# JaredWinkens/sdr-iq-visualizer

Measured on AMD Instinct MI355X. Metric: complex64 IQ Msamples/s through windowed FFT+log-PSD, N=4096; % HBM3E peak, higher is better.
Workload: dtype f32

## Files before the change

experiments/f4k_order/timeline.py:

```python
import argparse
import ctypes
import json
import os
import sys

REPO = os.path.dirname(os.path.dirname(os.path.dirname(os.path.abspath(__file__))))
sys.path.insert(0, REPO)
import torch
import numpy as np
from bench import warm_up_by_time
from sdr_iq_visualizer_amd import _ffi
from sdr_iq_visualizer_amd.spectrum import SpectrumPlan

NFFT = 4096
TICK_NS = 10.0
BIN_MS = 0.5


def analyse(rec, n_frames):
    t = rec[:, 0].astype(np.uint64) | (rec[:, 1].astype(np.uint64) << np.uint64(32))
    assert (t > 0).all(), "frames without a record"
    assert np.array_equal(rec[:, 2], np.arange(n_frames, dtype=np.uint32)), "a record names another frame than its own"
    wg = rec[:, 3].astype(np.int64)
    grid = int(wg.max()) + 1
# ... 7 lines not shown
    n_bins = int(np.ceil((ms.max() + 1e-9) / BIN_MS))
    cut = np.searchsorted(ms[order], np.arange(n_bins + 1) * BIN_MS, side="left")
    cut[-1] = n_frames
    for b in range(n_bins):
        hi = (b + 1) * BIN_MS
        idx = order[cut[b]:cut[b + 1]]
        if idx.size == 0:
            continue
        reached[wg[idx]] = frame[idx]
        active = (last_ms >= hi) & (reached >= 0)
        front = int(reached.max())
        lag = int(front - reached[active].min()) if active.any() else 0
        bins.append({"ms": round(b * BIN_MS, 2), "frames": int(idx.size), "span": int(frame[idx].max() - frame[idx].min()),
                     "lag_frames": lag, "lag_grids": round(lag / grid, 2)})
    return {"grid": grid, "launch_ms_by_records": round(float(ms.max()), 3), "bins": bins}


def main():
    ap = argparse.ArgumentParser()
    ap.add_argument("--out", required=True)
    ap.add_argument("--frames", type=int, default=1 << 20)
    ap.add_argument("--short", type=int, default=65536)
    ap.add_argument("--pairs", type=int, default=3)
    a = ap.parse_args()
    lib = _ffi.lib()
    _ffi.require_device(0)
    set_tl = lib.sdrk_f4k_timeline
    set_tl.argtypes, set_tl.restype = [ctypes.c_void_p], ctypes.c_int
    os.environ["SDRK_F4K_PARTS"] = "1"
    d_in = ctypes.c_void_p()
    _ffi.check(lib.sdrk_dev_alloc(0, a.frames * NFFT * 8, ctypes.byref(d_in)))
    outs = []
    for _ in range(a.pairs):
        p = ctypes.c_void_p()
        _ffi.check(lib.sdrk_dev_alloc(0, a.frames * NFFT * 4, ctypes.byref(p)))
        outs.append(p)
    _ffi.check(lib.sdrk_synth_fill(0, 1234, 0, a.frames, NFFT, d_in, None))
    tl = torch.zeros((a.frames, 4), dtype=torch.int32, device="cuda")
    os.makedirs(os.path.dirname(os.path.abspath(a.out)), exist_ok=True)
    with open(a.out, "a") as out:
        for order in ("stride", "ticket"):
            os.environ["SDRK_F4K_ORDER"] = order
            with SpectrumPlan(NFFT, window="hann", device=0) as plan:
                warm_up_by_time(lambda: plan.exec_device_timed(d_in.value, a.frames, outs[0].value, 1))
                for i, p in enumerate(outs):
                    for n in (a.frames, a.short):
                        plan.exec_device_timed(d_in.value, n, p.value, 1)
                        tl.zero_()
                        torch.cuda.synchronize()
                        assert set_tl(tl.data_ptr()) == 0
                        ms = plan.exec_device_timed(d_in.value, n, p.value, 1)
                        assert set_tl(None) == 0
                        rec = tl[:n].cpu().numpy().view(np.uint32)
                        r = {"order": order, "pair": i, "frames": n, "launch_ms_by_events": round(float(ms), 4), **analyse(rec, n)}
                        out.write(json.dumps(r) + "\n")
                        out.flush()
                        print(f"== {order} pair {i} frames {n}: {r['launch_ms_by_events']} ms by events, "
                              f"{r['launch_ms_by_records']} ms first to last issue, grid {r['grid']}")
                        for b in r["bins"]:
                            print(f"   {b['ms']:5.2f} ms  frames {b['frames']:7d}  span {b['span']:8d}  lag {b['lag_frames']:8d} "
                                  f"frames = {b['lag_grids']:7.2f} grids", flush=True)
    for p in outs:
        lib.sdrk_dev_free(0, p)
    lib.sdrk_dev_free(0, d_in)

# ... 4 lines not shown
```

sdr-iq-visualizer_amd/csrc/aux_kernels.hip:

```cpp
#include "kernels.h"
#include "synth_hash.h"

namespace sdrk {

__global__ __launch_bounds__(256) void synth_fill_kernel(uint32_t seed, uint64_t first_frame,
                                                         size_t n_frames, int nfft,
                                                         float4* __restrict__ out) {
    const size_t pairs_per_frame = (size_t)nfft / 2;
    const size_t total = n_frames * pairs_per_frame;
    for (size_t i = (size_t)blockIdx.x * blockDim.x + threadIdx.x; i < total;
         i += (size_t)gridDim.x * blockDim.x) {
        const size_t f = i / pairs_per_frame;
        const uint32_t n = (uint32_t)(i - f * pairs_per_frame) * 2u;
        const uint64_t F = first_frame + f;
        const uint32_t base = synth_frame_base(seed, F);
        int i0, q0, i1, q1;
        synth_codes(base, n, i0, q0);
        synth_codes(base, n + 1u, i1, q1);
        float4 v;
        v.x = (float)i0;
        v.y = (float)q0;
        v.z = (float)i1;
        v.w = (float)q1;
        out[i] = v;
// ... 112 lines not shown
__global__ __launch_bounds__(256) void copy_1to1_kernel(const v4f* __restrict__ in, v4f* __restrict__ out, size_t n_vec) {
    const size_t stride = (size_t)gridDim.x * 256 * 4;
    for (size_t i = (size_t)blockIdx.x * 1024 + threadIdx.x; i < n_vec; i += stride) {
        v4f v[4];
#pragma unroll
        for (int j = 0; j < 4; ++j)
            if (i + 256 * j < n_vec) v[j] = __builtin_nontemporal_load(&in[i + 256 * j]);
#pragma unroll
        for (int j = 0; j < 4; ++j)
            if (i + 256 * j < n_vec) __builtin_nontemporal_store(v[j], &out[i + 256 * j]);
    }
}

hipError_t launch_copy_1to1(const void* d_in, void* d_out, size_t bytes, int num_cus, int blocks_per_cu, hipStream_t stream) {
    const size_t n_vec = bytes / 16;
    if (n_vec == 0) return hipSuccess;
    size_t blocks = (n_vec + 1023) / 1024;
    if (blocks > (size_t)num_cus * blocks_per_cu) blocks = (size_t)num_cus * blocks_per_cu;
    hipLaunchKernelGGL(copy_1to1_kernel, dim3((unsigned)blocks), dim3(256), 0, stream, static_cast<const v4f*>(d_in),
                       static_cast<v4f*>(d_out), n_vec);
    return hipGetLastError();
}

hipError_t launch_power_mean(const void* d_spec, size_t n_frames, int nfft, float scale, float* d_out,
                             hipStream_t stream) {
    hipLaunchKernelGGL(power_mean_kernel, dim3((nfft + 255) / 256), dim3(256), 0, stream,
                       static_cast<const float2*>(d_spec), n_frames, nfft, scale, d_out);
    return hipGetLastError();
}

}
```

sdr-iq-visualizer_amd/csrc/fft4096.hip:

```cpp
#include "fft4096_core.h"

namespace sdrk {

#ifdef SDRK_F4K_TIMELINE
__device__ uint4* f4k_timeline_buf = nullptr;
#define F4K_TIMELINE_LOAD() uint4* const f4k_tl = f4k_timeline_buf
#define F4K_TIMELINE_MARK(fr)                                                                                   \
    do {                                                                                                        \
        if (f4k_tl && tid == 0 && (fr) < n_frames) {                                                            \
            const unsigned long long f4k_t = wall_clock64();                                                    \
            f4k_tl[fr] = make_uint4((unsigned)f4k_t, (unsigned)(f4k_t >> 32), (unsigned)(fr), blockIdx.x);      \
        }                                                                                                       \
    } while (0)
#else
#define F4K_TIMELINE_LOAD() (void)0
#define F4K_TIMELINE_MARK(fr) (void)0
#endif

template <bool HAS_WINDOW, int EPILOGUE>
__global__ __launch_bounds__(F4K_THREADS, F4K_WAVES) void fft4096_kernel(
    const float2* __restrict__ iq, size_t frame_stride, void* __restrict__ out_raw,
    size_t n_frames, const float* __restrict__ window, const float2* __restrict__ tw4096,
    float eps, int shift) {
    typedef F4kInC64 In;
// ... 94 lines not shown
        if (last_of_ticket && tid == 0) {
            ticket_slot[par] = drawn;
            drawn = __hip_atomic_fetch_add(head, 1u, __ATOMIC_RELAXED, __HIP_MEMORY_SCOPE_AGENT);
        }
        In::to_owners(nxt, lds, tid);
        cf v[16];
#pragma unroll
        for (int j = 0; j < 16; ++j) v[j] = In::widen(nxt[j]);
        issue(nxt, nx);
        f4k_windowed_transform<HAS_WINDOW>(v, lds, tw256, tw1, lds_win, A, tid);
        size_t after = nx + 1;
        if (last_of_ticket) {
            after = tn;
            tn = first_of(__builtin_amdgcn_readfirstlane(ticket_slot[par]));
            par ^= 1;
        }
        f4k_store_row<EPILOGUE>(v, frame_rsrc(static_cast<char*>(out_raw) + cur * (size_t)(F4K_N * OUT_ELEM), F4K_N * OUT_ELEM),
                                voff_out, xor_k2, eps);
        cur = nx;
        nx = after;
    }
}

unsigned f4k_max_blocks(int num_cus) { return f4k_grid(num_cus, F4K_WAVES, (size_t)-1); }

hipError_t launch_fft4096(const LaunchArgs& a) {
    if (a.n_frames == 0) return hipSuccess;
    dim3 g(f4k_grid(a.num_cus, F4K_WAVES, a.n_frames)), b(F4K_THREADS);
    const float2* iq = static_cast<const float2*>(a.d_iq);
    const float2* tw = static_cast<const float2*>(a.d_twiddle);
#define SDRK_LAUNCH(W, E)                                                                            \
    hipLaunchKernelGGL((fft4096_kernel<W, E>), g, b, 0, a.stream, iq, a.frame_stride, a.d_out,           \
                       a.n_frames, a.d_window, tw, a.eps, a.shift)
    if (a.epilogue == EPI_LOGPSD) {
        if (a.d_window) SDRK_LAUNCH(true, EPI_LOGPSD); else SDRK_LAUNCH(false, EPI_LOGPSD);
    } else {
        if (a.d_window) SDRK_LAUNCH(true, EPI_COMPLEX); else SDRK_LAUNCH(false, EPI_COMPLEX);
    }
#undef SDRK_LAUNCH
    return hipGetLastError();
}

hipError_t launch_fft4096_ticket(const LaunchArgs& a, unsigned* d_heads, const sdrk_host::F4kTicketBases& bases,
                                 sdrk_host::F4kTicketForm form, unsigned grid) {
    if (a.n_frames == 0) return hipSuccess;
    if (!d_heads || grid == 0 || grid % sdrk_host::F4K_TICKET_MAX_HEADS || !sdrk_host::f4k_ticket_form_ok(form)) return hipErrorInvalidValue;
    dim3 g(grid), b(F4K_THREADS);
    const float2* iq = static_cast<const float2*>(a.d_iq);
    const float2* tw = static_cast<const float2*>(a.d_twiddle);
#define SDRK_LAUNCH(W, E)                                                                            \
    hipLaunchKernelGGL((fft4096_ticket_kernel<W, E>), g, b, 0, a.stream, iq, a.frame_stride, a.d_out,    \
                       a.n_frames, a.d_window, tw, a.eps, a.shift, d_heads, bases, form)
    if (a.epilogue == EPI_LOGPSD) {
        if (a.d_window) SDRK_LAUNCH(true, EPI_LOGPSD); else SDRK_LAUNCH(false, EPI_LOGPSD);
    } else {
        if (a.d_window) SDRK_LAUNCH(true, EPI_COMPLEX); else SDRK_LAUNCH(false, EPI_COMPLEX);
    }
#undef SDRK_LAUNCH
    return hipGetLastError();
}

}

#ifdef SDRK_F4K_TIMELINE
extern "C" int sdrk_f4k_timeline(void* d_records) {
    uint4* p = static_cast<uint4*>(d_records);
    return (int)hipMemcpyToSymbol(HIP_SYMBOL(sdrk::f4k_timeline_buf), &p, sizeof p);
}
#endif
```

sdr-iq-visualizer_amd/csrc/kernels.h:

```cpp
#pragma once
#include <hip/hip_runtime.h>
#include <stddef.h>
#include <stdint.h>

#include <atomic>

#include "f4k_ticket.h"

#ifdef SDRK_PHASE_MARKS
#define SDRK_PHASE(name) asm volatile("; SDRK_PHASE " name ::: "memory")
#else
#define SDRK_PHASE(name) do { } while (0)
#endif

namespace sdrk {

enum Epilogue : int {
    EPI_LOGPSD = 0,
    EPI_COMPLEX = 1,
    EPI_BLU_MUL = 2,
    EPI_BLU_POST_LOG = 3,
    EPI_BLU_POST_C64 = 4,
};

struct LaunchArgs {
    const void* d_iq = nullptr;
    size_t frame_stride = 0;
    void* d_out = nullptr;
    size_t n_frames = 0;
    int nfft = 0;
// ... 26 lines not shown

__device__ __forceinline__ float logpsd_db_fast(float p) {
    return __builtin_amdgcn_logf(p) * 3.01029995663981195213f;
}

#endif

inline hipError_t ensure_dynamic_lds(const void* kernel, size_t lds_bytes, std::atomic<uint64_t>& mask) {
    if (lds_bytes <= 64 * 1024) return hipSuccess;
    int dev = 0;
    hipError_t e = hipGetDevice(&dev);
    if (e != hipSuccess) return e;
    const uint64_t bit = (dev >= 0 && dev < 64) ? (uint64_t)1 << dev : 0;
    if (bit && (mask.load(std::memory_order_acquire) & bit)) return hipSuccess;
    e = hipFuncSetAttribute(kernel, hipFuncAttributeMaxDynamicSharedMemorySize, (int)lds_bytes);
    if (e == hipSuccess && bit) mask.fetch_or(bit, std::memory_order_release);
    return e;
}

hipError_t launch_fft4096(const LaunchArgs& a);
unsigned f4k_max_blocks(int num_cus);
hipError_t launch_fft4096_ticket(const LaunchArgs& a, unsigned* d_heads, const sdrk_host::F4kTicketBases& bases,
                                 sdrk_host::F4kTicketForm form, unsigned grid);
hipError_t launch_fft_small(const LaunchArgs& a);
bool fft_lds_supports(int nfft);
hipError_t launch_fft_lds(const LaunchArgs& a);
bool fft_tiled2_split(int nfft, int* log2a, int* log2m);
hipError_t launch_fft_tiled2(const LaunchArgs& a);
bool fft_tiled2_has_mip(int nfft, int epilogue);
hipError_t launch_synth_fill(uint32_t seed, uint64_t first_frame, size_t n_frames, int nfft,
                             void* d_iq, hipStream_t stream);

size_t fused64k_ring_bytes();
size_t fused64k_ctrl_words();
unsigned fused64k_sets(int num_cus);
hipError_t launch_fused64k(const LaunchArgs& a, void* d_ring, unsigned* d_ctrl);
bool blu_fused_supports(int M);
hipError_t launch_blu_fused(const void* d_iq, size_t frame_stride, size_t n_frames, int N, int M, const float* d_window,
                            const void* d_chirp, const void* d_bspec, const void* d_twM, float eps, int shift,
                            int epilogue, void* d_out, int num_cus, hipStream_t s);
hipError_t launch_blu_pre(const void* d_iq, size_t frame_stride, size_t n_frames, int N, int M, const float* d_window,
                          const void* d_chirp, void* d_a, int num_cus, hipStream_t s, bool compact = false);
hipError_t launch_blu_mul(const void* d_A, const void* d_B, size_t n_frames, int M, void* d_out, int num_cus,
                          hipStream_t s);
hipError_t launch_blu_post(const void* d_Y, const void* d_chirp, size_t n_frames, int N, int M, float eps, int shift,
                           int epilogue, void* d_out, int num_cus, hipStream_t s);
hipError_t launch_row_features(const float* d_rows, size_t n_rows, int nfft, int rank, float gamma, int min_distance,
                               int max_peaks, double* d_stats, double* d_thr, int* d_idx, int* d_cnt, int num_cus,
                               hipStream_t s);
hipError_t launch_feature_finalize(const double* d_stats, const double* d_thr, const int* d_idx, const int* d_cnt,
                                   size_t n_rows, int nfft, float gamma, int max_peaks, const double* d_freqs,
                                   double* d_out, hipStream_t s);
hipError_t launch_fft4096_features(const LaunchArgs& a, int rank, float gamma, int min_distance, int max_peaks,
                                   double* d_stats, double* d_thr, int* d_idx, int* d_cnt);
hipError_t launch_row_peaks(const float* d_rows, size_t n_rows, int nfft, const double* d_thr, int min_distance,
                            int max_peaks, int* d_idx, int* d_count, hipStream_t s);
hipError_t launch_decimate_rows(const float* d_ring, int nfft, int maxlen, int start_slot, int n_rows, int factor,
                                int mode, float* d_out, hipStream_t stream);
hipError_t launch_decimate_mip(const float* d_mip_ring, int nfft, int maxlen, int start_slot, int n_rows, int factor,
                               float* d_out, hipStream_t stream);
hipError_t launch_stream_mix(const void* d_in, void* d_out, size_t n_frames4096, int num_cus, hipStream_t stream);
hipError_t launch_copy_1to1(const void* d_in, void* d_out, size_t bytes, int num_cus, int blocks_per_cu, hipStream_t stream);
hipError_t launch_power_mean(const void* d_spec, size_t n_frames, int nfft, float scale, float* d_out,
                             hipStream_t stream);

}
```

sdr-iq-visualizer_amd/csrc/plan_internal.h:

```cpp
#pragma once
#include <hip/hip_runtime.h>

#include <cstddef>
#include <cstdint>
#include <map>
#include <mutex>
#include <utility>
#include <vector>

#include "../../include/sdrk.h"
#include "kernels.h"

namespace sdrk_host {
constexpr int HOST_SLOTS = 3;
struct ChunkOut {
    enum Rows {
        None,
        Pooled,
        Direct,
        Kernel,
        Planes,
    } rows = None;
    void* user = nullptr;
    size_t bytes = 0;
// ... 67 lines not shown
    bool fused64k = false, fused_auto = false, fused_broken = false;
    void* d_fused_ring = nullptr;
    unsigned* d_fused_ctrl = nullptr;
    unsigned* h_fused_err = nullptr;
    unsigned fused_launches = 0, fused_pending = 0;
    int precision = 32;
    double eps64 = 0.0;
    double* d_window64 = nullptr;
    double* d_tw64 = nullptr;
    void* d_scratch64 = nullptr;
    sdrk_host::Staging ci16;
    sdrk_host::Staging integ;
    float* d_pfb_h = nullptr;
    int pfb_taps = 0;
    int pfb_assign = 0;
    sdrk_host::Staging pfb;
    float2* d_fir_h = nullptr;
    int fir_taps = 0;
    int fir_assign = 0;
    int f4k_order = sdrk_host::F4K_ORDER_AUTO;
    sdrk_host::F4kTicketForm f4k_form = sdrk_host::F4K_TICKET_FORM;
    unsigned* d_f4k_heads = nullptr;
    sdrk_host::F4kTicketBases f4k_bases = {};
    hipEvent_t f4k_ev = nullptr;
    hipStream_t f4k_last = nullptr;
    bool f4k_recorded = false;
    size_t f4k_parts = 0;
};

namespace sdrk_host {

constexpr size_t SMALL_IN_BYTES = 256 << 10;
constexpr size_t HOST_CHUNK_BYTES = 16 << 20;
constexpr size_t ZERO_COPY_MAX_BYTES = 32 << 20;
constexpr unsigned FUSED_MAILBOX = 64;
constexpr size_t FUSED_AUTO_MIN_FRAMES = 512;

int fail(int status, const char* fmt, ...) __attribute__((format(printf, 2, 3)));

#define HIP_TRY(expr)                                                                                                   \
    do {                                                                                                                \
        hipError_t e__ = (expr);                                                                                        \
        if (e__ != hipSuccess)                                                                                          \
            return ::sdrk_host::fail(e__ == hipErrorOutOfMemory ? SDRK_ERR_NOMEM : SDRK_ERR_HIP,                        \
                                     "%s failed: %s (%s:%d)", #expr, hipGetErrorString(e__), __FILE__, __LINE__);       \
    } while (0)
// ... 196 lines not shown
```

sdr-iq-visualizer_amd/csrc/sdrk_plan.hip:

```cpp
#include "../../include/sdrk.h"

#include <hip/hip_runtime.h>

#include <cmath>
#include <cstdio>
#include <cstdlib>
#include <cstring>
#include <dlfcn.h>
#include <mutex>
#include <new>
#include <vector>

#include "f4k_split.h"
#include "kernels.h"
#include "plan_internal.h"

using namespace sdrk_host;

namespace sdrk_host {

struct EpiArgs {
    const float2* tab = nullptr;
    int n_out = 0;
    float eps = 0.0f;
// ... 129 lines not shown
            if (st != SDRK_OK) return st;
            e = sdrk::launch_blu_mul(p->d_blu_b, p->d_blu_bspec, nf, M, p->d_blu_a, p->num_cus, stream);
            if (e != hipSuccess) break;
            st = plan_launch(p->blu_inner, p->d_blu_a, nf, (size_t)M, p->d_blu_b, sdrk::EPI_COMPLEX, stream);
            if (st != SDRK_OK) return st;
            e = sdrk::launch_blu_post(p->d_blu_b, p->d_blu_chirp, nf, N, M, p->eps, p->shift, epilogue,
                                      static_cast<char*>(d_out) + f0 * (size_t)N * out_elem, p->num_cus, stream);
            if (e != hipSuccess) break;
        }
    } else if (p->nfft == 4096) {
        const size_t max_blocks = sdrk::f4k_max_blocks(p->num_cus);
        const bool ticket = p->d_f4k_heads && f4k_ticket_takes(p->f4k_order, max_blocks, n_frames, F4K_TICKET_DEFAULT);
        size_t parts = p->f4k_parts ? p->f4k_parts : (ticket ? f4k_ticket_parts(n_frames) : f4k_split_parts(n_frames));
        if (p->f4k_parts && parts > n_frames) parts = n_frames ? n_frames : 1;
        const size_t per = (n_frames + parts - 1) / parts;
        const size_t out_elem = epilogue == sdrk::EPI_LOGPSD ? sizeof(float) : sizeof(float2);
        if (ticket && p->f4k_recorded && p->f4k_last != stream) e = hipStreamWaitEvent(stream, p->f4k_ev, 0);
        for (size_t f0 = 0; f0 < n_frames && e == hipSuccess; f0 += per) {
            a.d_iq = static_cast<const float2*>(d_iq) + f0 * frame_stride;
            a.d_out = static_cast<char*>(d_out) + f0 * (size_t)4096 * out_elem;
            a.n_frames = n_frames - f0 < per ? n_frames - f0 : per;
            if (ticket) {
                const unsigned grid = f4k_ticket_grid(max_blocks, a.n_frames);
                e = sdrk::launch_fft4096_ticket(a, p->d_f4k_heads, p->f4k_bases, p->f4k_form, grid);
                if (e == hipSuccess) f4k_ticket_advance(p->f4k_form, p->f4k_bases, a.n_frames, grid);
            } else {
                e = sdrk::launch_fft4096(a);
            }
        }
        if (ticket && e == hipSuccess) {
            e = hipEventRecord(p->f4k_ev, stream);
            p->f4k_last = stream;
            p->f4k_recorded = true;
        }
    } else if (sdrk::fft_lds_supports(p->nfft))
        e = sdrk::launch_fft_lds(a);
    else if (p->nfft < 4096)
        e = sdrk::launch_fft_small(a);
    else if (takes_fused(p, call_frames) && !d_mip && epilogue <= sdrk::EPI_COMPLEX) {
        FusedGate& gate = fused_gate(p->device);
        std::lock_guard<std::mutex> lk(gate.mu);
        if (gate.ev && gate.last_stream != stream && gate.recorded) e = hipStreamWaitEvent(stream, gate.ev, 0);
        if (e == hipSuccess) e = sdrk::launch_fused64k(a, p->d_fused_ring, p->d_fused_ctrl);
        if (e == hipSuccess)
            e = hipMemcpyAsync(p->h_fused_err + 16 * (p->fused_launches++ % FUSED_MAILBOX), p->d_fused_ctrl,
                               16 * sizeof(unsigned), hipMemcpyDeviceToHost, stream);
        if (e == hipSuccess && gate.ev) {
            e = hipEventRecord(gate.ev, stream);
// ... 163 lines not shown
            const double ang = M_PI * (double)r / (double)nfft;
            c[n] = make_float2((float)std::cos(ang), (float)std::sin(ang));
            b[n] = c[n];
            if (n) b[M - n] = c[n];
        }
        PLAN_TRY(hipMalloc((void**)&p->d_blu_chirp, sizeof(float2) * nfft));
        PLAN_TRY(hipMemcpy(p->d_blu_chirp, c.data(), sizeof(float2) * nfft, hipMemcpyHostToDevice));
        PLAN_TRY(hipMalloc((void**)&p->d_blu_a, (one_kernel ? 1 : frames) * (size_t)M * sizeof(float2)));
        if (!one_kernel) PLAN_TRY(hipMalloc((void**)&p->d_blu_b, frames * (size_t)M * sizeof(float2)));
        PLAN_TRY(hipMalloc((void**)&p->d_blu_bspec, (size_t)M * sizeof(float2)));
        PLAN_TRY(hipMemcpy(p->d_blu_a, b.data(), sizeof(float2) * M, hipMemcpyHostToDevice));
        st2 = plan_launch(p->blu_inner, p->d_blu_a, 1, (size_t)M, p->d_blu_bspec, sdrk::EPI_COMPLEX, p->stream);
        if (st2 != SDRK_OK) { sdrk_plan_destroy(p); return st2; }
        PLAN_TRY(hipStreamSynchronize(p->stream));
        *out = p;
        return SDRK_OK;
    }
    if (nfft <= 16384) {
        std::vector<float2> t(nfft);
        for (int m = 0; m < nfft; ++m) t[m] = twiddle(m, nfft);
        PLAN_TRY(hipMalloc((void**)&p->d_twiddle, sizeof(float2) * nfft));
        PLAN_TRY(hipMemcpy(p->d_twiddle, t.data(), sizeof(float2) * nfft, hipMemcpyHostToDevice));
        if (nfft == 4096) {
            if (const char* env = getenv("SDRK_F4K_ORDER"))
                p->f4k_order = env[0] == 't' ? F4K_ORDER_TICKET : (env[0] == 's' ? F4K_ORDER_STRIDE : F4K_ORDER_AUTO);
            if (const char* env = getenv("SDRK_F4K_PARTS")) {
                long v = atol(env);
                if (v >= 1 && v <= 4096) p->f4k_parts = (size_t)v;
            }
            if (const char* env = getenv("SDRK_F4K_TICKET_FORM")) {
                F4kTicketForm f = {0, 0};
                if (sscanf(env, "%ux%u", &f.heads, &f.frames) == 2 && f4k_ticket_form_ok(f)) p->f4k_form = f;
            }
            std::vector<uint32_t> h(F4K_TICKET_MAX_HEADS * F4K_TICKET_HEAD_WORDS, 0u);
            for (unsigned x = 0; x < F4K_TICKET_MAX_HEADS; ++x) h[x * F4K_TICKET_HEAD_WORDS] = p->f4k_bases.base[x] = 0xFFFFFE00u;
            PLAN_TRY(hipMalloc((void**)&p->d_f4k_heads, h.size() * sizeof(uint32_t)));
            PLAN_TRY(hipMemcpy(p->d_f4k_heads, h.data(), h.size() * sizeof(uint32_t), hipMemcpyHostToDevice));
            PLAN_TRY(hipEventCreateWithFlags(&p->f4k_ev, hipEventDisableTiming));
        }
    } else {
        size_t scratch_mb = 192;
        if (const char* env = getenv("SDRK_SCRATCH_MB")) {
            long v = atol(env);
            if (v >= 1 && v <= 65536) scratch_mb = (size_t)v;
        }
        size_t frames = (scratch_mb << 20) / ((size_t)nfft * sizeof(float2));
        if (frames < 1) frames = 1;
        if (frames > max_batch) frames = max_batch;
        p->scratch_frames = frames;
        PLAN_TRY(hipMalloc((void**)&p->d_scratch, frames * (size_t)nfft * sizeof(float2)));
        int la = 0, lm = 0;
        if (!sdrk::fft_tiled2_split(nfft, &la, &lm)) {
            sdrk_plan_destroy(p);
            return fail(SDRK_ERR_UNSUPPORTED, "no kernel for nfft=%d", nfft);
        }
        const int A = 1 << la, M = 1 << lm, TA = A / 16;
// ... 72 lines not shown
    if (p->d_tw_2p) (void)hipFree(p->d_tw_2p);
    if (p->d_scratch) (void)hipFree(p->d_scratch);
    if (p->blu_inner) (void)sdrk_plan_destroy(p->blu_inner);
    if (p->d_blu_chirp) (void)hipFree(p->d_blu_chirp);
    if (p->d_blu_bspec) (void)hipFree(p->d_blu_bspec);
    if (p->d_blu_a) (void)hipFree(p->d_blu_a);
    if (p->d_blu_b) (void)hipFree(p->d_blu_b);
    if (p->h_small_in) (void)hipHostFree(p->h_small_in);
    if (p->h_small_out) (void)hipHostFree(p->h_small_out);
    if (p->h_small_flag) (void)hipHostFree(p->h_small_flag);
    if (p->d_fused_ring) (void)hipFree(p->d_fused_ring);
    if (p->d_fused_ctrl) (void)hipFree(p->d_fused_ctrl);
    if (p->h_fused_err) (void)hipHostFree(p->h_fused_err);
    if (p->d_in) (void)hipFree(p->d_in);
    if (p->d_out) (void)hipFree(p->d_out);
    if (p->d_feat) (void)hipFree(p->d_feat);
    p->ci16.release();
    p->integ.release();
    if (p->d_pfb_h) (void)hipFree(p->d_pfb_h);
    p->pfb.release();
    if (p->d_fir_h) (void)hipFree(p->d_fir_h);
    if (p->f4k_recorded) (void)hipEventSynchronize(p->f4k_ev);
    if (p->d_f4k_heads) (void)hipFree(p->d_f4k_heads);
    if (p->f4k_ev) (void)hipEventDestroy(p->f4k_ev);
    if (p->s_h2d) (void)hipStreamSynchronize(p->s_h2d);
    if (p->s_d2h) (void)hipStreamSynchronize(p->s_d2h);
    for (auto& sl : p->slot) {
        if (sl.h_in) (void)hipHostFree(sl.h_in);
        if (sl.h_out) (void)hipHostFree(sl.h_out);
        if (sl.d_in) (void)hipFree(sl.d_in);
        if (sl.d_out) (void)hipFree(sl.d_out);
        if (sl.ev_in) (void)hipEventDestroy(sl.ev_in);
        if (sl.ev_k) (void)hipEventDestroy(sl.ev_k);
        if (sl.ev_done) (void)hipEventDestroy(sl.ev_done);
    }
    if (p->s_h2d) (void)hipStreamDestroy(p->s_h2d);
    if (p->s_d2h) (void)hipStreamDestroy(p->s_d2h);
    if (p->ev0) (void)hipEventDestroy(p->ev0);
    if (p->ev1) (void)hipEventDestroy(p->ev1);
    if (p->stream) (void)hipStreamDestroy(p->stream);
    delete p;
    return SDRK_OK;
}

int sdrk_plan_nfft(const sdrk_plan* p) { return p ? p->nfft : fail(SDRK_ERR_INVALID, "plan is NULL"); }
int sdrk_plan_device(const sdrk_plan* p) { return p ? p->device : fail(SDRK_ERR_INVALID, "plan is NULL"); }
// ... 37 lines not shown
```

sdr-iq-visualizer_amd/csrc/sdrk_probes.hip:

```cpp
#include "../../include/sdrk.h"

#include <hip/hip_runtime.h>

#include <algorithm>
#include <chrono>
#include <cstring>
#include <vector>

#include "kernels.h"
#include "plan_internal.h"

using namespace sdrk_host;

namespace sdrk_host {
namespace {

thread_local int g_probe_status = SDRK_OK;
hipError_t probe_launch_result(int st) {
    if (st == SDRK_OK) return hipSuccess;
    g_probe_status = st;
    return hipErrorUnknown;
}
int probe_fail(hipError_t e, const char* what) {
    if (e == hipErrorUnknown && g_probe_status != SDRK_OK) {
// ... 55 lines not shown
    if (st != SDRK_OK) return st;
    HIP_TRY(hipSetDevice(device));
    hipDeviceProp_t prop;
    HIP_TRY(hipGetDeviceProperties(&prop, device));
    hipStream_t s = nullptr;
    hipEvent_t e0 = nullptr, e1 = nullptr;
    HIP_TRY(hipStreamCreateWithFlags(&s, hipStreamNonBlocking));
    hipError_t e = hipEventCreate(&e0);
    if (e == hipSuccess) e = hipEventCreate(&e1);
    for (int i = -2; i < launches && e == hipSuccess; ++i) {
        if (i >= 0) e = hipEventRecord(e0, s);
        if (e == hipSuccess) e = launch(prop.multiProcessorCount, s);
        if (i >= 0 && e == hipSuccess) e = hipEventRecord(e1, s);
        if (i >= 0 && e == hipSuccess) e = hipEventSynchronize(e1);
        if (i >= 0 && e == hipSuccess) e = hipEventElapsedTime(&each_ms[i], e0, e1);
    }
    (void)hipStreamSynchronize(s);
    if (e0) (void)hipEventDestroy(e0);
    if (e1) (void)hipEventDestroy(e1);
    (void)hipStreamDestroy(s);
    if (e != hipSuccess) return fail(SDRK_ERR_HIP, "%s failed: %s", what, hipGetErrorString(e));
    return SDRK_OK;
}

}

int tune_staging(sdrk_plan* p) {
    const size_t nfft = (size_t)p->nfft;
    if (p->blu_inner || p->max_batch * nfft * sizeof(float2) <= 2 * HOST_CHUNK_BYTES) return SDRK_OK;
    size_t per = HOST_CHUNK_BYTES / (nfft * sizeof(float2));
    if (per < 1) per = 1;
    const size_t in_b = per * nfft * sizeof(float2), out_b = per * nfft * sizeof(float);
    hipEvent_t e0 = nullptr, e1 = nullptr;
    HIP_TRY(hipEventCreate(&e0));
    if (hipError_t ee = hipEventCreate(&e1); ee != hipSuccess) {
        (void)hipEventDestroy(e0);
        return fail(SDRK_ERR_HIP, "hipEventCreate failed: %s", hipGetErrorString(ee));
    }
    int st = SDRK_OK;
    PlacementReport rep;
    for (int i = 0; i < HOST_SLOTS && st == SDRK_OK; ++i) {
        HostSlot& s = p->slot[i];
        st = slot_reserve(p, s, in_b, 0);
        if (st != SDRK_OK) break;
        if (hipHostMalloc(&s.h_out, out_b, hipHostMallocDefault) != hipSuccess) { st = fail(SDRK_ERR_NOMEM, "pinned staging"); break; }
        void* cand[3] = {nullptr, nullptr, nullptr};
// ... 179 lines not shown
    if (probe_ms) for (int c = n_ok; c < candidates; ++c) probe_ms[c] = 0.0f;
    if (chosen) *chosen = best;
    rep.candidates = n_ok;
    rep.chosen = best;
    g_placement = rep;
    if (e != hipSuccess) return probe_fail(e, "scratch placement probe failed");
    return fused_check(p);
}

int sdrk_placement_report(float* warm_ms, int* warm_launches, float* first_ms, float* retimed_first_ms, float* chosen_ms) {
    const PlacementReport& r = g_placement;
    if (warm_ms) *warm_ms = r.warm_ms;
    if (warm_launches) *warm_launches = r.warm_launches;
    if (first_ms) *first_ms = r.first_ms;
    if (retimed_first_ms) *retimed_first_ms = r.retimed_first_ms;
    if (chosen_ms) *chosen_ms = r.chosen_ms;
    return r.candidates;
}

int sdrk_stream_ceiling_probe(int device, const void* d_in, void* d_out, size_t n_frames4096, int launches,
                              float* each_ms) {
    if (!d_in || !d_out || !each_ms || launches < 1 || launches > 4096 || n_frames4096 == 0)
        return fail(SDRK_ERR_INVALID, "bad argument");
    return timed_probe(device, launches, each_ms, "stream ceiling probe", [&](int cus, hipStream_t s) {
        return sdrk::launch_stream_mix(d_in, d_out, n_frames4096, cus, s);
    });
}

int sdrk_copy_probe(int device, const void* d_in, void* d_out, size_t bytes, int launches, float* each_ms) {
    if (!d_in || !d_out || !each_ms || launches < 1 || launches > 4096 || bytes < 16)
        return fail(SDRK_ERR_INVALID, "bad argument");
    std::vector<float> t((size_t)launches), best;
    float best_med = 0.0f;
    for (int bpc : {3, 4, 16}) {
        int st = timed_probe(device, launches, t.data(), "copy probe", [&](int cus, hipStream_t s) {
            return sdrk::launch_copy_1to1(d_in, d_out, bytes, cus, bpc, s);
        });
        if (st != SDRK_OK) return st;
        std::vector<float> sorted = t;
        std::sort(sorted.begin(), sorted.end());
        const float med = sorted[sorted.size() / 2];
        if (best.empty() || med < best_med) { best = t; best_med = med; }
    }
    memcpy(each_ms, best.data(), sizeof(float) * (size_t)launches);
    return SDRK_OK;
}

int sdrk_host_link_probe(int device, size_t bytes, double* h2d_gbps, double* d2h_gbps, double* duplex_gbps) {
    if (!h2d_gbps || !d2h_gbps || !duplex_gbps || bytes < (1u << 20)) return fail(SDRK_ERR_INVALID, "bad argument");
    int st = check_device(device);
    if (st != SDRK_OK) return st;
    HIP_TRY(hipSetDevice(device));
    void *h_a = nullptr, *h_b = nullptr, *d_a = nullptr, *d_b = nullptr;
    hipStream_t s0 = nullptr, s1 = nullptr;
    hipEvent_t e0 = nullptr, e1 = nullptr, e2 = nullptr;
    hipError_t e = hipHostMalloc(&h_a, bytes, hipHostMallocDefault);
    if (e == hipSuccess) e = hipHostMalloc(&h_b, bytes / 2, hipHostMallocDefault);
    if (e == hipSuccess) e = hipMalloc(&d_a, bytes);
    if (e == hipSuccess) e = hipMalloc(&d_b, bytes / 2);
// ... 56 lines not shown
```

Measured before the change: 514,400.

## Add rotating multi-head ticket dealer for FFT4096 frame scheduling

Adds a rotating-head work dealer: each workgroup pulls frame tickets from several atomic counters in turn, and the last workgroup to exit resets the counters so no host-side base bookkeeping is needed between launches. The 4096-point FFT ticket path now defaults to this dealer with four heads when ticket order is chosen, and the bandwidth probes use the same dealer. The aim is to cut contention on a single ticket counter and keep frame issue order tight across workgroups. The cost is extra atomics per frame, LDS handoff slots, and a reset step on exit.

```diff
diff --git a/experiments/f4k_order/timeline.py b/experiments/f4k_order/timeline.py
--- a/experiments/f4k_order/timeline.py
+++ b/experiments/f4k_order/timeline.py
@@ -53,6 +53,8 @@
     ap.add_argument("--frames", type=int, default=1 << 20)
     ap.add_argument("--short", type=int, default=65536)
     ap.add_argument("--pairs", type=int, default=3)
+    ap.add_argument("--orders", default="stride,ticket",
+                    help="comma-separated SDRK_F4K_ORDER values, each optionally with :<SDRK_F4K_TICKET_FORM> (ticket:rot4)")
     a = ap.parse_args()
     lib = _ffi.lib()
     _ffi.require_device(0)
@@ -70,8 +72,12 @@
     tl = torch.zeros((a.frames, 4), dtype=torch.int32, device="cuda")
     os.makedirs(os.path.dirname(os.path.abspath(a.out)), exist_ok=True)
     with open(a.out, "a") as out:
-        for order in ("stride", "ticket"):
-            os.environ["SDRK_F4K_ORDER"] = order
+        for order in [o for o in a.orders.split(",") if o]:
+            os.environ["SDRK_F4K_ORDER"] = order.split(":")[0]
+            if ":" in order:
+                os.environ["SDRK_F4K_TICKET_FORM"] = order.split(":")[1]
+            else:
+                os.environ.pop("SDRK_F4K_TICKET_FORM", None)
             with SpectrumPlan(NFFT, window="hann", device=0) as plan:
                 warm_up_by_time(lambda: plan.exec_device_timed(d_in.value, a.frames, outs[0].value, 1))
                 for i, p in enumerate(outs):
diff --git a/sdr-iq-visualizer_amd/csrc/aux_kernels.hip b/sdr-iq-visualizer_amd/csrc/aux_kernels.hip
--- a/sdr-iq-visualizer_amd/csrc/aux_kernels.hip
+++ b/sdr-iq-visualizer_amd/csrc/aux_kernels.hip
@@ -1,3 +1,4 @@
+#include "f4k_deal.h"
 #include "kernels.h"
 #include "synth_hash.h"
 
@@ -158,6 +159,100 @@
     return hipGetLastError();
 }
 
+template <class Deal>
+__global__ __launch_bounds__(256) void stream_mix_dealt_kernel(const v4f* __restrict__ in, v4f* __restrict__ out, size_t n_frames,
+                                                               const sdrk_host::F4kDealArgs da) {
+    __shared__ unsigned deal_slot[F4K_DEAL_SLOTS];
+    const int tid = threadIdx.x;
+    Deal deal = Deal::make(da, n_frames, deal_slot, tid);
+    deal.publish(tid);
+    __syncthreads();
+    deal.begin();
+    while (deal.more()) {
+        deal.top(tid);
+        const size_t f = deal.frame();
+        if (f < n_frames) {
+            const v4f* x = in + f * 2048;
+            v4f* o = out + f * 1024;
+            v4f v[8];
+#pragma unroll
+            for (int j = 0; j < 8; ++j) v[j] = __builtin_nontemporal_load(&x[tid + 256 * j]);
+#pragma unroll
+            for (int j = 0; j < 4; ++j) __builtin_nontemporal_store(v[2 * j] + v[2 * j + 1], &o[tid + 256 * j]);
+        }
+        __syncthreads();
+        deal.step();
+    }
+    deal.leave(tid);
+}
+
+template <class Deal>
+__global__ __launch_bounds__(256) void copy_1to1_dealt_kernel(const v4f* __restrict__ in, v4f* __restrict__ out, size_t n_vec,
+                                                              const sdrk_host::F4kDealArgs da) {
+    __shared__ unsigned deal_slot[F4K_DEAL_SLOTS];
+    const int tid = threadIdx.x;
+    const size_t n_units = (n_vec + 1023) / 1024;
+    Deal deal = Deal::make(da, n_units, deal_slot, tid);
+    deal.publish(tid);
+    __syncthreads();
+    deal.begin();
+    while (deal.more()) {
+        deal.top(tid);
+        const size_t u = deal.frame();
+        if (u < n_units) {
+            const size_t i = u * 1024 + tid;
+            v4f v[4];
+#pragma unroll
+            for (int j = 0; j < 4; ++j)
+                if (i + 256 * j < n_vec) v[j] = __builtin_nontemporal_load(&in[i + 256 * j]);
+#pragma unroll
+            for (int j = 0; j < 4; ++j)
+                if (i + 256 * j < n_vec) __builtin_nontemporal_store(v[j], &out[i + 256 * j]);
+        }
+        __syncthreads();
+        deal.step();
+    }
+    deal.leave(tid);
+}
+
+template <class Launch>
+static hipError_t launch_dealt(sdrk_host::F4kProbeDeal& pd, size_t max_blocks, size_t n_units, Launch&& launch) {
+    using namespace sdrk_host;
+    if (!pd.d_heads || !f4k_ticket_takes(pd.choice.order, max_blocks, n_units, F4K_TICKET_DEFAULT)) return hipErrorNotSupported;
+    const unsigned grid = f4k_ticket_grid(max_blocks, n_units);
+    const F4kDealArgs da = {pd.d_heads, pd.bases, pd.choice.form, pd.choice.rot_heads};
+    launch(grid, da, pd.choice.rot_heads != 0);
+    const hipError_t e = hipGetLastError();
+    if (e == hipSuccess && !pd.choice.rot_heads) f4k_ticket_advance(pd.choice.form, pd.bases, n_units, grid);
+    return e;
+}
+
+hipError_t launch_stream_mix_dealt(const void* d_in, void* d_out, size_t n_frames4096, int num_cus, hipStream_t stream,
+                                   sdrk_host::F4kProbeDeal& pd) {
+    if (n_frames4096 == 0) return hipSuccess;
+    const v4f* in = static_cast<const v4f*>(d_in);
+    v4f* out = static_cast<v4f*>(d_out);
+    const hipError_t e = launch_dealt(pd, (size_t)num_cus * 3, n_frames4096, [&](unsigned grid, const sdrk_host::F4kDealArgs& da, bool rot) {
+        if (rot) hipLaunchKernelGGL(stream_mix_dealt_kernel<F4kRotDeal>, dim3(grid), dim3(256), 0, stream, in, out, n_frames4096, da);
+        else hipLaunchKernelGGL(stream_mix_dealt_kernel<F4kTicketDeal>, dim3(grid), dim3(256), 0, stream, in, out, n_frames4096, da);
+    });
+    return e == hipErrorNotSupported ? launch_stream_mix(d_in, d_out, n_frames4096, num_cus, stream) : e;
+}
+
+hipError_t launch_copy_1to1_dealt(const void* d_in, void* d_out, size_t bytes, int num_cus, int blocks_per_cu, hipStream_t stream,
+                                  sdrk_host::F4kProbeDeal& pd) {
+    const size_t n_vec = bytes / 16;
+    if (n_vec == 0) return hipSuccess;
+    const v4f* in = static_cast<const v4f*>(d_in);
+    v4f* out = static_cast<v4f*>(d_out);
+    const hipError_t e = launch_dealt(pd, (size_t)num_cus * blocks_per_cu, (n_vec + 1023) / 1024,
+                                      [&](unsigned grid, const sdrk_host::F4kDealArgs& da, bool rot) {
+        if (rot) hipLaunchKernelGGL(copy_1to1_dealt_kernel<F4kRotDeal>, dim3(grid), dim3(256), 0, stream, in, out, n_vec, da);
+        else hipLaunchKernelGGL(copy_1to1_dealt_kernel<F4kTicketDeal>, dim3(grid), dim3(256), 0, stream, in, out, n_vec, da);
+    });
+    return e == hipErrorNotSupported ? launch_copy_1to1(d_in, d_out, bytes, num_cus, blocks_per_cu, stream) : e;
+}
+
 hipError_t launch_power_mean(const void* d_spec, size_t n_frames, int nfft, float scale, float* d_out,
                              hipStream_t stream) {
     hipLaunchKernelGGL(power_mean_kernel, dim3((nfft + 255) / 256), dim3(256), 0, stream,
diff --git a/sdr-iq-visualizer_amd/csrc/f4k_deal.h b/sdr-iq-visualizer_amd/csrc/f4k_deal.h
--- /dev/null
+++ b/sdr-iq-visualizer_amd/csrc/f4k_deal.h
@@ -0,0 +1,137 @@
+#pragma once
+#include <hip/hip_runtime.h>
+
+#include "f4k_rot.h"
+#include "f4k_ticket.h"
+
+namespace sdrk {
+
+constexpr int F4K_DEAL_SLOTS = 4;
+
+__device__ __forceinline__ unsigned f4k_deal_draw(unsigned* word, unsigned n) {
+    return __hip_atomic_fetch_add(word, n, __ATOMIC_RELAXED, __HIP_MEMORY_SCOPE_AGENT);
+}
+
+struct F4kTicketDeal {
+    sdrk_host::F4kTicketForm form;
+    size_t n_frames, cur, nx, tn, in_ticket;
+    unsigned* head;
+    unsigned* slot;
+    unsigned hx, base, depth, drawn, par;
+    bool last_of_ticket;
+
+    __device__ __forceinline__ F4kTicketDeal(unsigned* heads, const sdrk_host::F4kTicketBases& bases, sdrk_host::F4kTicketForm f,
+                                             size_t n, unsigned* lds_slots, int tid)
+        : form(f), n_frames(n), in_ticket(f.frames - 1), slot(lds_slots), hx(blockIdx.x & (f.heads - 1)),
+          depth(sdrk_host::f4k_ticket_depth(f)), drawn(0), par(1), last_of_ticket(false) {
+        head = heads + hx * sdrk_host::F4K_TICKET_HEAD_WORDS + __lane_id();
+        base = bases.base[hx];
+        if (tid == 0) drawn = f4k_deal_draw(head, depth);
+    }
+    static __device__ __forceinline__ F4kTicketDeal make(const sdrk_host::F4kDealArgs& a, size_t n, unsigned* lds_slots, int tid) {
+        return F4kTicketDeal(a.heads, a.bases, a.form, n, lds_slots, tid);
+    }
+    __device__ __forceinline__ size_t first_of(unsigned head_value) const {
+        return sdrk_host::f4k_ticket_first_frame(form, head_value - base, hx);
+    }
+    __device__ __forceinline__ void publish(int tid) {
+        if (tid == 0) {
+            slot[0] = drawn;
+            drawn += depth - 1;
+        }
+    }
+    __device__ __forceinline__ void begin() {
+        const unsigned h0 = __builtin_amdgcn_readfirstlane(slot[0]);
+        cur = first_of(h0);
+        nx = in_ticket ? cur + 1 : first_of(h0 + 1);
+        tn = first_of(h0 + depth - 2);
+    }
+    __device__ __forceinline__ bool more() const { return cur < n_frames; }
+    __device__ __forceinline__ void top(int tid) {
+        last_of_ticket = ((nx + 1) & in_ticket) == 0;
+        if (last_of_ticket && tid == 0) {
+            slot[par] = drawn;
+            drawn = f4k_deal_draw(head, 1u);
+        }
+    }
+    __device__ __forceinline__ size_t frame() const { return cur; }
+    __device__ __forceinline__ size_t next() const { return nx; }
+    __device__ __forceinline__ void step() {
+        size_t after = nx + 1;
+        if (last_of_ticket) {
+            after = tn;
+            tn = first_of(__builtin_amdgcn_readfirstlane(slot[par]));
+            par ^= 1;
+        }
+        cur = nx;
+        nx = after;
+    }
+    __device__ __forceinline__ void leave(int) {}
+};
+
+struct F4kRotDeal {
+    sdrk_host::F4kRotDrawer dr;
+    size_t n_frames;
+    unsigned* lane_heads;
+    unsigned* slot;
+    unsigned drawn, d0, d1, h0, h1;
+    unsigned cur, nx, par;
+
+    __device__ __forceinline__ F4kRotDeal(unsigned* heads, unsigned n_heads, size_t n, unsigned* lds_slots, int tid)
+        : dr(sdrk_host::f4k_rot_drawer(n_heads, blockIdx.x)), n_frames(n), lane_heads(heads + __lane_id()), slot(lds_slots),
+          drawn(0), d0(0), d1(0), h0(0), h1(0), par(2) {
+        if (tid == 0) {
+            h0 = dr.head;
+            d0 = f4k_deal_draw(word(h0), 1u);
+            h1 = (h0 + 1) & (n_heads - 1);
+            d1 = f4k_deal_draw(word(h1), 1u);
+            dr.head = (h1 + 1) & (n_heads - 1);
+            drawn = f4k_deal_draw(word(dr.head), 1u);
+            dr.pending = true;
+        }
+    }
+    static __device__ __forceinline__ F4kRotDeal make(const sdrk_host::F4kDealArgs& a, size_t n, unsigned* lds_slots, int tid) {
+        return F4kRotDeal(a.heads, a.rot_heads, n, lds_slots, tid);
+    }
+    __device__ __forceinline__ unsigned* word(unsigned head) const { return lane_heads + head * sdrk_host::F4K_TICKET_HEAD_WORDS; }
+    __device__ __forceinline__ void publish(int tid) {
+        if (tid == 0) {
+            const unsigned h2 = dr.head;
+            dr.head = h0;
+            slot[0] = sdrk_host::f4k_rot_take(dr, d0, n_frames);
+            dr.head = h1;
+            slot[1] = sdrk_host::f4k_rot_take(dr, d1, n_frames);
+            dr.head = h2;
+        }
+    }
+    __device__ __forceinline__ void begin() {
+        cur = __builtin_amdgcn_readfirstlane(slot[0]);
+        nx = __builtin_amdgcn_readfirstlane(slot[1]);
+    }
+    __device__ __forceinline__ bool more() const { return cur != sdrk_host::F4K_ROT_NONE; }
+    __device__ __forceinline__ void top(int tid) {
+        if (tid == 0) {
+            slot[par] = dr.pending ? sdrk_host::f4k_rot_take(dr, drawn, n_frames) : sdrk_host::F4K_ROT_NONE;
+            if (sdrk_host::f4k_rot_advance(dr)) drawn = f4k_deal_draw(word(dr.head), 1u);
+        }
+    }
+    __device__ __forceinline__ size_t frame() const { return cur; }
+    __device__ __forceinline__ size_t next() const { return nx; }
+    __device__ __forceinline__ void step() {
+        const unsigned after = __builtin_amdgcn_readfirstlane(slot[par]);
+        par ^= 1;
+        cur = nx;
+        nx = after;
+    }
+    __device__ __forceinline__ void leave(int tid) {
+        if (tid == 0) {
+            unsigned* const exits = lane_heads + sdrk_host::F4K_ROT_EXIT_WORD;
+            if (f4k_deal_draw(exits, 1u) == gridDim.x - 1) {
+                for (unsigned x = 0; x < dr.heads; ++x) __hip_atomic_store(word(x), 0u, __ATOMIC_RELAXED, __HIP_MEMORY_SCOPE_AGENT);
+                __hip_atomic_store(exits, 0u, __ATOMIC_RELAXED, __HIP_MEMORY_SCOPE_AGENT);
+            }
+        }
+    }
+};
+
+}
diff --git a/sdr-iq-visualizer_amd/csrc/f4k_rot.h b/sdr-iq-visualizer_amd/csrc/f4k_rot.h
--- /dev/null
+++ b/sdr-iq-visualizer_amd/csrc/f4k_rot.h
@@ -0,0 +1,81 @@
+#pragma once
+#include <cstddef>
+#include <cstdint>
+#include <cstdio>
+
+#include "f4k_ticket.h"
+
+namespace sdrk_host {
+
+constexpr unsigned F4K_ROT_AHEAD = 3;
+constexpr unsigned F4K_ROT_EXIT_WORD = F4K_TICKET_MAX_HEADS * F4K_TICKET_HEAD_WORDS;
+constexpr unsigned F4K_ROT_WORDS = (F4K_TICKET_MAX_HEADS + 1) * F4K_TICKET_HEAD_WORDS;
+constexpr uint32_t F4K_ROT_NONE = 0xFFFFFFFFu;
+
+constexpr bool f4k_rot_heads_ok(unsigned heads) { return heads == 2 || heads == 4 || heads == 8; }
+
+constexpr uint32_t f4k_rot_frame(unsigned heads, uint32_t ticket, unsigned head) { return ticket * heads + head; }
+
+constexpr unsigned f4k_rot_next_head(unsigned heads, unsigned live, unsigned last) {
+    const unsigned twice = live | (live << heads);
+    return (last + 1 + (unsigned)__builtin_ctz(twice >> (last + 1))) & (heads - 1);
+}
+
+struct F4kRotDrawer {
+    unsigned heads;
+    unsigned live;
+    unsigned head;
+    bool pending;
+};
+constexpr F4kRotDrawer f4k_rot_drawer(unsigned heads, unsigned workgroup) {
+    return F4kRotDrawer{heads, (1u << heads) - 1u, workgroup & (heads - 1), false};
+}
+constexpr uint32_t f4k_rot_take(F4kRotDrawer& d, uint32_t ticket, size_t n_frames) {
+    const uint32_t fr = f4k_rot_frame(d.heads, ticket, d.head);
+    if (fr >= n_frames) d.live &= ~(1u << d.head);
+    return fr;
+}
+constexpr bool f4k_rot_advance(F4kRotDrawer& d) {
+    d.pending = d.live != 0;
+    if (d.pending) d.head = f4k_rot_next_head(d.heads, d.live, d.head);
+    return d.pending;
+}
+
+inline unsigned f4k_rot_parse(const char* s) {
+    if (!s || s[0] != 'r' || s[1] != 'o' || s[2] != 't' || s[3] == 0 || s[4] != 0) return 0;
+    const unsigned h = (unsigned)(s[3] - '0');
+    return f4k_rot_heads_ok(h) ? h : 0;
+}
+
+constexpr unsigned F4K_ROT_DEFAULT_HEADS = 4;
+
+struct F4kChoice {
+    int order = F4K_ORDER_AUTO;
+    F4kTicketForm form = F4K_TICKET_FORM;
+    unsigned rot_heads = F4K_ROT_DEFAULT_HEADS;
+};
+inline F4kChoice f4k_choice(const char* order_env, const char* form_env) {
+    F4kChoice c;
+    if (order_env) c.order = order_env[0] == 't' ? F4K_ORDER_TICKET : (order_env[0] == 's' ? F4K_ORDER_STRIDE : F4K_ORDER_AUTO);
+    if (form_env) {
+        F4kTicketForm f = {0, 0};
+        if (const unsigned rot = f4k_rot_parse(form_env)) c.rot_heads = rot;
+        else if (sscanf(form_env, "%ux%u", &f.heads, &f.frames) == 2 && f4k_ticket_form_ok(f)) { c.form = f; c.rot_heads = 0; }
+    }
+    return c;
+}
+
+struct F4kDealArgs {
+    unsigned* heads;
+    F4kTicketBases bases;
+    F4kTicketForm form;
+    unsigned rot_heads;
+};
+
+struct F4kProbeDeal {
+    F4kChoice choice;
+    unsigned* d_heads = nullptr;
+    F4kTicketBases bases = {};
+};
+
+}
diff --git a/sdr-iq-visualizer_amd/csrc/fft4096.hip b/sdr-iq-visualizer_amd/csrc/fft4096.hip
--- a/sdr-iq-visualizer_amd/csrc/fft4096.hip
+++ b/sdr-iq-visualizer_amd/csrc/fft4096.hip
@@ -1,3 +1,4 @@
+#include "f4k_deal.h"
 #include "fft4096_core.h"
 
 namespace sdrk {
@@ -140,6 +141,64 @@
     }
 }
 
+template <bool HAS_WINDOW, int EPILOGUE>
+__global__ __launch_bounds__(F4K_THREADS, F4K_WAVES) void fft4096_rot_kernel(
+    const float2* __restrict__ iq, size_t frame_stride, void* __restrict__ out_raw,
+    size_t n_frames, const float* __restrict__ window, const float2* __restrict__ tw4096,
+    float eps, int shift, unsigned* __restrict__ heads, const unsigned n_heads) {
+    typedef F4kInC64 In;
+    __shared__ float2 lds[f4k_lds_elems(HAS_WINDOW)];
+    __shared__ unsigned deal_slot[F4K_DEAL_SLOTS];
+    float2* __restrict__ tw256 = lds + F4K_XCH_ELEMS;
+    float2* __restrict__ tw1 = tw256 + 256;
+    float* __restrict__ lds_win = reinterpret_cast<float*>(tw1 + 256);
+
+    const int tid = threadIdx.x;
+    F4kRotDeal deal(heads, n_heads, n_frames, deal_slot, tid);
+    F4kAddr A = f4k_addr(tid);
+    f4k_init_tables(tw256, tw1, tw4096, tid);
+    if (HAS_WINDOW) {
+#pragma unroll
+        for (int j = 0; j < 16; ++j) lds_win[tid + 256 * j] = window[tid + 256 * j];
+    }
+    deal.publish(tid);
+    __syncthreads();
+
+    const int xor_k2 = shift ? 8 : 0;
+    constexpr int OUT_ELEM = (EPILOGUE == EPI_LOGPSD ? 4 : 8);
+    const int voff_out = tid * OUT_ELEM;
+    F4K_TIMELINE_LOAD();
+
+    auto issue = [&](In::word (&x)[16], size_t fr) {
+        F4K_TIMELINE_MARK(fr);
+        if (fr >= n_frames) fr = 0;
+        In::issue(x, iq + fr * frame_stride, tid);
+    };
+    In::word nxt[16];
+    deal.begin();
+    issue(nxt, deal.frame());
+    while (deal.more()) {
+        deal.top(tid);
+        const size_t cur = deal.frame();
+        if (cur < n_frames) {
+            In::to_owners(nxt, lds, tid);
+            cf v[16];
+#pragma unroll
+            for (int j = 0; j < 16; ++j) v[j] = In::widen(nxt[j]);
+            issue(nxt, deal.next());
+            f4k_windowed_transform<HAS_WINDOW>(v, lds, tw256, tw1, lds_win, A, tid);
+            deal.step();
+            f4k_store_row<EPILOGUE>(v, frame_rsrc(static_cast<char*>(out_raw) + cur * (size_t)(F4K_N * OUT_ELEM), F4K_N * OUT_ELEM),
+                                    voff_out, xor_k2, eps);
+        } else {
+            issue(nxt, deal.next());
+            __syncthreads();
+            deal.step();
+        }
+    }
+    deal.leave(tid);
+}
+
 unsigned f4k_max_blocks(int num_cus) { return f4k_grid(num_cus, F4K_WAVES, (size_t)-1); }
 
 hipError_t launch_fft4096(const LaunchArgs& a) {
@@ -178,6 +237,26 @@
     return hipGetLastError();
 }
 
+hipError_t launch_fft4096_rot(const LaunchArgs& a, unsigned* d_heads, unsigned n_heads, unsigned grid) {
+    if (a.n_frames == 0) return hipSuccess;
+    if (!d_heads || grid == 0 || grid % sdrk_host::F4K_TICKET_MAX_HEADS || !sdrk_host::f4k_rot_heads_ok(n_heads) ||
+        a.n_frames > sdrk_host::F4K_TICKET_MAX_FRAMES)
+        return hipErrorInvalidValue;
+    dim3 g(grid), b(F4K_THREADS);
+    const float2* iq = static_cast<const float2*>(a.d_iq);
+    const float2* tw = static_cast<const float2*>(a.d_twiddle);
+#define SDRK_LAUNCH(W, E)                                                                            \
+    hipLaunchKernelGGL((fft4096_rot_kernel<W, E>), g, b, 0, a.stream, iq, a.frame_stride, a.d_out,       \
+                       a.n_frames, a.d_window, tw, a.eps, a.shift, d_heads, n_heads)
+    if (a.epilogue == EPI_LOGPSD) {
+        if (a.d_window) SDRK_LAUNCH(true, EPI_LOGPSD); else SDRK_LAUNCH(false, EPI_LOGPSD);
+    } else {
+        if (a.d_window) SDRK_LAUNCH(true, EPI_COMPLEX); else SDRK_LAUNCH(false, EPI_COMPLEX);
+    }
+#undef SDRK_LAUNCH
+    return hipGetLastError();
+}
+
 }
 
 #ifdef SDRK_F4K_TIMELINE
diff --git a/sdr-iq-visualizer_amd/csrc/kernels.h b/sdr-iq-visualizer_amd/csrc/kernels.h
--- a/sdr-iq-visualizer_amd/csrc/kernels.h
+++ b/sdr-iq-visualizer_amd/csrc/kernels.h
@@ -6,6 +6,7 @@
 #include <atomic>
 
 #include "f4k_ticket.h"
+#include "f4k_rot.h"
 
 #ifdef SDRK_PHASE_MARKS
 #define SDRK_PHASE(name) asm volatile("; SDRK_PHASE " name ::: "memory")
@@ -78,6 +79,7 @@
 unsigned f4k_max_blocks(int num_cus);
 hipError_t launch_fft4096_ticket(const LaunchArgs& a, unsigned* d_heads, const sdrk_host::F4kTicketBases& bases,
                                  sdrk_host::F4kTicketForm form, unsigned grid);
+hipError_t launch_fft4096_rot(const LaunchArgs& a, unsigned* d_heads, unsigned n_heads, unsigned grid);
 hipError_t launch_fft_small(const LaunchArgs& a);
 bool fft_lds_supports(int nfft);
 hipError_t launch_fft_lds(const LaunchArgs& a);
@@ -117,6 +119,10 @@
                                float* d_out, hipStream_t stream);
 hipError_t launch_stream_mix(const void* d_in, void* d_out, size_t n_frames4096, int num_cus, hipStream_t stream);
 hipError_t launch_copy_1to1(const void* d_in, void* d_out, size_t bytes, int num_cus, int blocks_per_cu, hipStream_t stream);
+hipError_t launch_stream_mix_dealt(const void* d_in, void* d_out, size_t n_frames4096, int num_cus, hipStream_t stream,
+                                   sdrk_host::F4kProbeDeal& pd);
+hipError_t launch_copy_1to1_dealt(const void* d_in, void* d_out, size_t bytes, int num_cus, int blocks_per_cu, hipStream_t stream,
+                                  sdrk_host::F4kProbeDeal& pd);
 hipError_t launch_power_mean(const void* d_spec, size_t n_frames, int nfft, float scale, float* d_out,
                              hipStream_t stream);
 
diff --git a/sdr-iq-visualizer_amd/csrc/plan_internal.h b/sdr-iq-visualizer_amd/csrc/plan_internal.h
--- a/sdr-iq-visualizer_amd/csrc/plan_internal.h
+++ b/sdr-iq-visualizer_amd/csrc/plan_internal.h
@@ -113,6 +113,8 @@
     sdrk_host::F4kTicketForm f4k_form = sdrk_host::F4K_TICKET_FORM;
     unsigned* d_f4k_heads = nullptr;
     sdrk_host::F4kTicketBases f4k_bases = {};
+    unsigned f4k_rot_heads = sdrk_host::F4K_ROT_DEFAULT_HEADS;
+    unsigned* d_f4k_rot = nullptr;
     hipEvent_t f4k_ev = nullptr;
     hipStream_t f4k_last = nullptr;
     bool f4k_recorded = false;
diff --git a/sdr-iq-visualizer_amd/csrc/sdrk_plan.hip b/sdr-iq-visualizer_amd/csrc/sdrk_plan.hip
--- a/sdr-iq-visualizer_amd/csrc/sdrk_plan.hip
+++ b/sdr-iq-visualizer_amd/csrc/sdrk_plan.hip
@@ -175,8 +175,12 @@
             a.n_frames = n_frames - f0 < per ? n_frames - f0 : per;
             if (ticket) {
                 const unsigned grid = f4k_ticket_grid(max_blocks, a.n_frames);
-                e = sdrk::launch_fft4096_ticket(a, p->d_f4k_heads, p->f4k_bases, p->f4k_form, grid);
-                if (e == hipSuccess) f4k_ticket_advance(p->f4k_form, p->f4k_bases, a.n_frames, grid);
+                if (p->f4k_rot_heads) {
+                    e = sdrk::launch_fft4096_rot(a, p->d_f4k_rot, p->f4k_rot_heads, grid);
+                } else {
+                    e = sdrk::launch_fft4096_ticket(a, p->d_f4k_heads, p->f4k_bases, p->f4k_form, grid);
+                    if (e == hipSuccess) f4k_ticket_advance(p->f4k_form, p->f4k_bases, a.n_frames, grid);
+                }
             } else {
                 e = sdrk::launch_fft4096(a);
             }
@@ -386,16 +390,17 @@
         PLAN_TRY(hipMalloc((void**)&p->d_twiddle, sizeof(float2) * nfft));
         PLAN_TRY(hipMemcpy(p->d_twiddle, t.data(), sizeof(float2) * nfft, hipMemcpyHostToDevice));
         if (nfft == 4096) {
-            if (const char* env = getenv("SDRK_F4K_ORDER"))
-                p->f4k_order = env[0] == 't' ? F4K_ORDER_TICKET : (env[0] == 's' ? F4K_ORDER_STRIDE : F4K_ORDER_AUTO);
+            const F4kChoice choice = f4k_choice(getenv("SDRK_F4K_ORDER"), getenv("SDRK_F4K_TICKET_FORM"));
+            p->f4k_order = choice.order;
+            p->f4k_form = choice.form;
+            p->f4k_rot_heads = choice.rot_heads;
             if (const char* env = getenv("SDRK_F4K_PARTS")) {
                 long v = atol(env);
                 if (v >= 1 && v <= 4096) p->f4k_parts = (size_t)v;
             }
-            if (const char* env = getenv("SDRK_F4K_TICKET_FORM")) {
-                F4kTicketForm f = {0, 0};
-                if (sscanf(env, "%ux%u", &f.heads, &f.frames) == 2 && f4k_ticket_form_ok(f)) p->f4k_form = f;
-            }
+            PLAN_TRY(hipMalloc((void**)&p->d_f4k_rot, F4K_ROT_WORDS * sizeof(uint32_t)));
+            const std::vector<uint32_t> rot0(F4K_ROT_WORDS, 0u);
+            PLAN_TRY(hipMemcpy(p->d_f4k_rot, rot0.data(), rot0.size() * sizeof(uint32_t), hipMemcpyHostToDevice));
             std::vector<uint32_t> h(F4K_TICKET_MAX_HEADS * F4K_TICKET_HEAD_WORDS, 0u);
             for (unsigned x = 0; x < F4K_TICKET_MAX_HEADS; ++x) h[x * F4K_TICKET_HEAD_WORDS] = p->f4k_bases.base[x] = 0xFFFFFE00u;
             PLAN_TRY(hipMalloc((void**)&p->d_f4k_heads, h.size() * sizeof(uint32_t)));
@@ -514,6 +519,7 @@
     if (p->d_fir_h) (void)hipFree(p->d_fir_h);
     if (p->f4k_recorded) (void)hipEventSynchronize(p->f4k_ev);
     if (p->d_f4k_heads) (void)hipFree(p->d_f4k_heads);
+    if (p->d_f4k_rot) (void)hipFree(p->d_f4k_rot);
     if (p->f4k_ev) (void)hipEventDestroy(p->f4k_ev);
     if (p->s_h2d) (void)hipStreamSynchronize(p->s_h2d);
     if (p->s_d2h) (void)hipStreamSynchronize(p->s_d2h);
diff --git a/sdr-iq-visualizer_amd/csrc/sdrk_probes.hip b/sdr-iq-visualizer_amd/csrc/sdrk_probes.hip
--- a/sdr-iq-visualizer_amd/csrc/sdrk_probes.hip
+++ b/sdr-iq-visualizer_amd/csrc/sdrk_probes.hip
@@ -101,6 +101,27 @@
     if (e != hipSuccess) return fail(SDRK_ERR_HIP, "%s failed: %s", what, hipGetErrorString(e));
     return SDRK_OK;
 }
+
+struct ProbeHeads {
+    F4kProbeDeal deal;
+    int status = SDRK_OK;
+    explicit ProbeHeads(int device) {
+        deal.choice = f4k_choice(getenv("SDRK_F4K_ORDER"), getenv("SDRK_F4K_TICKET_FORM"));
+        if (deal.choice.order == F4K_ORDER_STRIDE) return;
+        status = check_device(device);
+        if (status != SDRK_OK) return;
+        const std::vector<uint32_t> zero(F4K_ROT_WORDS, 0u);
+        hipError_t e = hipSetDevice(device);
+        if (e == hipSuccess) e = hipMalloc((void**)&deal.d_heads, zero.size() * sizeof(uint32_t));
+        if (e == hipSuccess) e = hipMemcpy(deal.d_heads, zero.data(), zero.size() * sizeof(uint32_t), hipMemcpyHostToDevice);
+        if (e != hipSuccess) status = fail(SDRK_ERR_HIP, "probe heads: %s", hipGetErrorString(e));
+    }
+    ~ProbeHeads() {
+        if (deal.d_heads) (void)hipFree(deal.d_heads);
+    }
+    ProbeHeads(const ProbeHeads&) = delete;
+    ProbeHeads& operator=(const ProbeHeads&) = delete;
+};
 
 }
 
@@ -326,8 +347,10 @@
                               float* each_ms) {
     if (!d_in || !d_out || !each_ms || launches < 1 || launches > 4096 || n_frames4096 == 0)
         return fail(SDRK_ERR_INVALID, "bad argument");
+    ProbeHeads heads(device);
+    if (heads.status != SDRK_OK) return heads.status;
     return timed_probe(device, launches, each_ms, "stream ceiling probe", [&](int cus, hipStream_t s) {
-        return sdrk::launch_stream_mix(d_in, d_out, n_frames4096, cus, s);
+        return sdrk::launch_stream_mix_dealt(d_in, d_out, n_frames4096, cus, s, heads.deal);
     });
 }
 
@@ -336,9 +359,11 @@
         return fail(SDRK_ERR_INVALID, "bad argument");
     std::vector<float> t((size_t)launches), best;
     float best_med = 0.0f;
+    ProbeHeads heads(device);
+    if (heads.status != SDRK_OK) return heads.status;
     for (int bpc : {3, 4, 16}) {
         int st = timed_probe(device, launches, t.data(), "copy probe", [&](int cus, hipStream_t s) {
-            return sdrk::launch_copy_1to1(d_in, d_out, bytes, cus, bpc, s);
+            return sdrk::launch_copy_1to1_dealt(d_in, d_out, bytes, cus, bpc, s, heads.deal);
         });
         if (st != SDRK_OK) return st;
         std::vector<float> sorted = t;
```

Result: faster. 527,800, median of 6 (+2.6%).
